# psy-ex/svt-av1-psy

Hardware: NVIDIA B200
Metric: 1080p preset-8 encoded frames/sec at 1/2/4/8 B200 vs reference AVX2 on host (higher is better)
Workload: dtype u8

## Files before the change

svt-av1-psy_b200/csrc/wiener.cu:

```cuda
#include <cuda_fp16.h>

#include <map>

#include "common.cuh"
#include "wiener_unit.cuh"
#include "../../include/svt_b200.h"
#include "wiener_stats_lag.cuh"

namespace b200 {


template <typename PIX>
__global__ void __launch_bounds__(256)
wiener_convolve_kernel(const PIX* __restrict__ src_base, PIX* __restrict__ dst_base, const SvtB200WienerUnit* __restrict__ units,
                       int n_units, int bd, int round0, int round1, int lbd_rows) {
    __shared__ __align__(16) uint16_t s_src[(64 + 8) * (64 + 8)];
    __shared__ __align__(16) uint16_t s_tmp[(64 + 8) * 64];
    for (int it = blockIdx.x; it < n_units; it += gridDim.x) {
        const SvtB200WienerUnit u = units[it];
        const int w = u.w, h = u.h;
        const PIX* src = src_base + u.src_off;
        PIX*       dst = dst_base + u.dst_off;
        const int sw = w + 8, sh = h + 7;
#pragma unroll 4
        for (int i = threadIdx.x; i < sw * sh; i += blockDim.x) {
            const int r = i / sw, c = i - r * sw;
            s_src[r * 72 + c] = (uint16_t)src[(ptrdiff_t)(r - 3) * u.src_stride + (c - 3)];
        }
        __syncthreads();
        wiener_unit_compute<PIX>(s_src, s_tmp, dst, u.dst_stride, w, h, u.hfilter, u.vfilter, bd, round0, round1, lbd_rows);
    }
}

constexpr int kSumParts = 16;
template <typename PIX>
__global__ void __launch_bounds__(256)
stats_sum_kernel(const PIX* __restrict__ dgd_base, const SvtB200StatsItem* __restrict__ items, unsigned long long* __restrict__ tot_out) {
    const int it = blockIdx.x / kSumParts, part = blockIdx.x % kSumParts;
    const SvtB200StatsItem s = items[it];
    const int w = s.h_end - s.h_start, h = s.v_end - s.v_start;
    const int warp = threadIdx.x >> 5, lane = threadIdx.x & 31;
    unsigned int acc = 0;
    unsigned long long wide = 0;
    for (int r = part * 8 + warp; r < h; r += kSumParts * 8) {
        const PIX* row = dgd_base + s.dgd_off + (ptrdiff_t)(s.v_start + r) * s.dgd_stride + s.h_start;
        for (int c = lane; c < w; c += 32) acc += row[c];
        if (acc > 0xf0000000u) { wide += acc; acc = 0; }
    }
    wide += acc;
#pragma unroll
    for (int o = 16; o > 0; o >>= 1) wide += __shfl_xor_sync(0xffffffffu, wide, o);
    if (lane == 0 && wide) atomicAdd(&tot_out[it], wide);
}

__device__ __forceinline__ int stats_average(const unsigned long long* tot, int it, const SvtB200StatsItem& s) {
    return (int)(tot[it] / (unsigned long long)((s.h_end - s.h_start) * (s.v_end - s.v_start)));
}

constexpr int kStatsMaxParts = 32;


constexpr int kMmaWarps = 4;
constexpr int kMmaTW = 64, kMmaTH = 32;
constexpr int kMmaPitch = 100;
constexpr int kMmaPRows = kMmaTH + 8;
constexpr int kMmaXBase = kMmaPRows * kMmaPitch + 28;
constexpr int kMmaWords = kMmaXBase + kMmaTH * kMmaPitch;
constexpr int kMmaAccMax = 16 * 128;
constexpr int kMmaFoldPixels = 33025 - kMmaTW * kMmaTH;
static_assert(kMmaPitch % 32 == 4 && (kMmaPRows * kMmaPitch) % 32 == 0, "bank layout");
static_assert(kMmaTW + 6 <= kMmaPitch && kMmaAccMax <= 2450, "layout");

__device__ __forceinline__ void mma_16816_f16f32(float (&c)[4], uint32_t a0, uint32_t a1, uint32_t a2, uint32_t a3, uint32_t b0,
                                                 uint32_t b1) {
    asm volatile("mma.sync.aligned.m16n8k16.row.col.f32.f16.f16.f32 {%0,%1,%2,%3}, {%4,%5,%6,%7}, {%8,%9}, {%0,%1,%2,%3};\n"
                 : "+f"(c[0]), "+f"(c[1]), "+f"(c[2]), "+f"(c[3])
                 : "r"(a0), "r"(a1), "r"(a2), "r"(a3), "r"(b0), "r"(b1));
}

__device__ __forceinline__ uint32_t pack_pair_f16(int lo, int hi) {
    const uint32_t bits = 0x64006400u + (uint32_t)(lo + 256) + ((uint32_t)(hi + 256) << 16);
    const __half2  h    = __hsub2(*reinterpret_cast<const __half2*>(&bits), __float2half2_rn(1280.f));
    return *reinterpret_cast<const uint32_t*>(&h);
}

__host__ __device__ __forceinline__ int mma_tile_index(int win, int m, int n) { return m * win - m * (m - 1) + n - 2 * m; }
__device__ __forceinline__ int stats_mma_parts(const SvtB200StatsItem& s, int ctas_per_item) {
    const int tiles = ((s.h_end - s.h_start + kMmaTW - 1) / kMmaTW) * ((s.v_end - s.v_start + kMmaTH - 1) / kMmaTH);
    return tiles < ctas_per_item ? tiles : ctas_per_item;
}

template <int WIN>
__device__ __forceinline__ void stats_mma_body(const uint8_t* __restrict__ dgd, const uint8_t* __restrict__ src, const SvtB200StatsItem& s,
                                               const int avg, const int part, const int parts, long long* __restrict__ P,
                                               uint32_t* __restrict__ tile, int* __restrict__ s32) {
    constexpr int NT = WIN, MT = (WIN + 1) / 2, HALF = WIN / 2, OFF = 3 - HALF;
    constexpr int NTILES = MT * WIN - MT * (MT - 1);
    const int warp = threadIdx.x >> 5, lane = threadIdx.x & 31, g = lane >> 2, t = lane & 3;
    int boff[NT];
#pragma unroll
    for (int n = 0; n < NT; n++) boff[n] = (OFF + g) * kMmaPitch + OFF + n + t;
    if (g == 7) boff[0] = kMmaXBase + t;
    float acc[NTILES][4];
#pragma unroll
    for (int i = 0; i < NTILES; i++) acc[i][0] = acc[i][1] = acc[i][2] = acc[i][3] = 0.f;
    for (int i = threadIdx.x; i < NTILES * 128; i += kMmaWarps * 32) s32[i] = 0;
    __syncthreads();
    auto flush_regs = [&]() {
#pragma unroll
        for (int i = 0; i < NTILES; i++)
#pragma unroll
            for (int r = 0; r < 4; r++) {
                atomicAdd(&s32[(i * 4 + r) * 32 + lane], __float2int_rn(acc[i][r]));
                acc[i][r] = 0.f;
            }
    };
    const int W = s.h_end - s.h_start, H = s.v_end - s.v_start;
    const int ntx = (W + kMmaTW - 1) / kMmaTW, nty = (H + kMmaTH - 1) / kMmaTH;
    const int vlo = s.v_start - HALF, vhi = s.v_end + HALF, hlo = s.h_start - HALF, hhi = s.h_end + HALF;
    int  ksteps = 0, pending = 0;
    bool spilled = false;
    auto prefetch_tile = [&](int tl) {
        const int ty = tl / ntx, tx = tl - ty * ntx;
        const int r0 = s.v_start + ty * kMmaTH, c0 = s.h_start + tx * kMmaTW;
        for (int w = threadIdx.x; w < 2 * (kMmaPRows + 1) + kMmaTH; w += kMmaWarps * 32) {
            const uint8_t* p;
            if (w < 2 * (kMmaPRows + 1)) {
                const int row = min(max(r0 - 3 + (w >> 1), vlo), vhi - 1);
                const int col = (w & 1) ? min(c0 + kMmaTW + 2, hhi - 1) : max(c0 - 3, hlo);
                p = dgd + (ptrdiff_t)row * s.dgd_stride + col;
            } else {
                const int row = min(r0 + (w - 2 * (kMmaPRows + 1)), s.v_end - 1);
                p = src + (ptrdiff_t)row * s.src_stride + min(c0 + 32, s.h_end - 1);
            }
            asm volatile("prefetch.global.L1 [%0];" ::"l"(p));
        }
    };
    for (int tl = part; tl < ntx * nty; tl += parts) {
        const int ty = tl / ntx, tx = tl - ty * ntx;
        const int r0 = s.v_start + ty * kMmaTH, c0 = s.h_start + tx * kMmaTW;
        const int nrows = min(kMmaTH, s.v_end - r0), ncols = min(kMmaTW, s.h_end - c0);
        if (pending > kMmaFoldPixels) {
            flush_regs();
            ksteps = 0;
            __syncthreads();
            for (int i = threadIdx.x; i < NTILES * 128; i += kMmaWarps * 32) {
                P[i] = (spilled ? P[i] : 0) + s32[i];
                s32[i] = 0;
            }
            spilled = true;
            pending = 0;
        }
        __syncthreads();
        for (int w = threadIdx.x; w < (kMmaTW + 6) * 4; w += kMmaWarps * 32) {
            const int  seg = w / (kMmaTW + 6), c = w - seg * (kMmaTW + 6);
            const int  col = c0 - 3 + c;
            const bool cv = col >= hlo && col < hhi;
            const int  rbeg = seg * (kMmaPRows / 4);
            auto ld = [&](int rr) {
                const int row = r0 - 3 + rr;
                return (cv && row >= vlo && row < vhi) ? (int)dgd[(ptrdiff_t)row * s.dgd_stride + col] - avg : 0;
            };
            int lo = ld(rbeg);
#pragma unroll
            for (int k = 0; k < kMmaPRows / 4; k++) {
                const int hi = ld(rbeg + k + 1);
                tile[(rbeg + k) * kMmaPitch + c] = pack_pair_f16(lo, hi);
                lo = hi;
            }
        }
        for (int w = threadIdx.x; w < (kMmaTH / 2) * kMmaTW; w += kMmaWarps * 32) {
            const int  r = (w / kMmaTW) * 2, c = w % kMmaTW;
            const bool cv = c < ncols;
            const uint8_t* p = src + (ptrdiff_t)(r0 + r) * s.src_stride + c0 + c;
            const int lo = (cv && r < nrows) ? (int)p[0] - avg : 0;
            const int hi = (cv && r + 1 < nrows) ? (int)p[s.src_stride] - avg : 0;
            tile[kMmaXBase + r * kMmaPitch + c] = pack_pair_f16(lo, hi);
        }
        __syncthreads();
        if (tl + parts < ntx * nty) prefetch_tile(tl + parts);
        const int cgs = (ncols + 7) >> 3, nsteps = cgs * ((nrows + 1) >> 1);
        for (int st = warp; st < nsteps; st += kMmaWarps) {
            const int rp = st / cgs, px = (st - rp * cgs) * 8, py = rp * 2;
            const uint32_t* base = tile + py * kMmaPitch + px;
            const uint32_t rowmask = (py + 1 < nrows) ? 0xffffffffu : 0x0000ffffu;
            const uint32_t m0 = (px + t < ncols) ? rowmask : 0u, m1 = (px + t + 4 < ncols) ? rowmask : 0u;
            uint32_t f0[NT], f1[NT];
#pragma unroll
            for (int n = 0; n < NT; n++) {
                f0[n] = base[boff[n]];
                f1[n] = base[boff[n] + 4];
            }
#pragma unroll
            for (int m = 0; m < MT; m++) {
                constexpr int last = NT - 1;
                const int     lo = 2 * m, hi = 2 * m + 1 <= last ? 2 * m + 1 : last;
#pragma unroll
                for (int n = 2 * m; n < NT; n++)
                    mma_16816_f16f32(acc[m * WIN - m * (m - 1) + n - 2 * m], f0[lo], f0[hi], f1[lo], f1[hi], f0[n] & m0, f1[n] & m1);
            }
            if (++ksteps == 16) {
                flush_regs();
                ksteps = 0;
            }
        }
        pending += nrows * ncols;
    }
    flush_regs();
    __syncthreads();
    for (int i = threadIdx.x; i < NTILES * 128; i += kMmaWarps * 32) P[i] = (spilled ? P[i] : 0) + s32[i];
}

__global__ void __launch_bounds__(kMmaWarps * 32)
stats_mma_kernel(const uint8_t* __restrict__ dgd_base, const uint8_t* __restrict__ src_base, const SvtB200StatsItem* __restrict__ items,
                 const unsigned long long* __restrict__ tot_in, int ctas_per_item, long long* __restrict__ partial) {
    __shared__ uint32_t tile[kMmaWords];
    __shared__ int      s32[kMmaAccMax];
    const int it = blockIdx.x / ctas_per_item, part = blockIdx.x % ctas_per_item;
    const SvtB200StatsItem s = items[it];
    const int avg = stats_average(tot_in, it, s);
    if (part >= stats_mma_parts(s, ctas_per_item)) return;
    long long* P = partial + ((size_t)it * ctas_per_item + part) * 2450;
    const uint8_t* dgd = dgd_base + s.dgd_off;
    const uint8_t* src = src_base + s.src_off;
    if (s.wiener_win == 7) stats_mma_body<7>(dgd, src, s, avg, part, ctas_per_item, P, tile, s32);
    else if (s.wiener_win == 5) stats_mma_body<5>(dgd, src, s, avg, part, ctas_per_item, P, tile, s32);
    else stats_mma_body<3>(dgd, src, s, avg, part, ctas_per_item, P, tile, s32);
}

__global__ void __launch_bounds__(256)
stats_finalize_kernel(const long long* __restrict__ partial, int parts, const SvtB200StatsItem* __restrict__ items, int divider,
                      int mma_layout, long long* __restrict__ M_out, long long* __restrict__ H_out) {
    const int it = blockIdx.y, e = blockIdx.x * blockDim.x + threadIdx.x;
    const int win = items[it].wiener_win, win2 = win * win;
    if (e >= win2 * win2 + win2) return;
    const int used = mma_layout ? stats_mma_parts(items[it], parts) : parts;
    int       src;
    if (e < win2 * win2) {
        const int k = e / win2, l = e - k * win2;
        int ka = k / win, kq = k - ka * win, la = l / win, lq = l - la * win;
        if (mma_layout) {
            if (ka > la) {
                int x = ka; ka = la; la = x;
                x = kq; kq = lq; lq = x;
            }
            src = (mma_tile_index(win, ka >> 1, la) * 4 + (ka & 1) * 2 + (lq & 1)) * 32 + kq * 4 + (lq >> 1);
        } else {
            src = (ka <= la) ? k * win2 + l : l * win2 + k;
        }
    } else {
        const int k = e - win2 * win2, ka = k / win, kq = k - ka * win;
        src = mma_layout ? (mma_tile_index(win, 0, ka) * 4 + (kq & 1)) * 32 + 28 + (kq >> 1) : 2401 + k;
    }
    long long v = 0;
    for (int p = 0; p < used; p++) v += partial[((size_t)it * parts + p) * 2450 + src];
    if (e < win2 * win2) H_out[(size_t)it * 2401 + e] = v / divider;
    else M_out[(size_t)it * 49 + (e - win2 * win2)] = v / divider;
}

struct StatsScratch {
    long long*          acc = nullptr;
    unsigned long long* tot = nullptr;
    size_t              cap = 0;
};
static std::map<cudaStream_t, StatsScratch> g_stats;
static std::mutex g_stats_mu;
static ResetHook g_stats_reset([] { std::lock_guard<std::mutex> lk(g_stats_mu); g_stats.clear(); });

template <typename PIX, int WIN>
static void launch_lag_bulk(const PIX* d_dgd, const PIX* d_src, const SvtB200StatsItem* d_items, int n, int cpi, unsigned long long* acc,
                            cudaStream_t st) {
    constexpr size_t smem = lag_bulk_smem<PIX, WIN>();
    static int attr = -1;
    if (attr != epoch()) {
        if (smem > 48 * 1024)
            B200_CUDA_CHECK(cudaFuncSetAttribute(stats_lag_bulk_kernel<PIX, WIN>, cudaFuncAttributeMaxDynamicSharedMemorySize, (int)smem));
        attr = epoch();
    }
    stats_lag_bulk_kernel<PIX, WIN><<<dim3(cpi, n), 256, smem, st>>>(d_dgd, d_src, d_items, acc);
    B200_LAUNCH_CHECK();
}

template <typename PIX>
static void launch_stats_mma(const PIX* d_dgd, const PIX* d_src, const SvtB200StatsItem* d_items, int n, int bd, long long* d_M,
                             long long* d_H, long long* d_acc, unsigned long long* d_tot, cudaStream_t st);

template <typename PIX>
static void launch_stats(const PIX* d_dgd, const PIX* d_src, const SvtB200StatsItem* d_items, int n, int bd, long long* d_M,
                         long long* d_H, long long* d_acc, unsigned long long* d_tot, cudaStream_t st) {
    if constexpr (sizeof(PIX) == 1) return launch_stats_mma<PIX>(d_dgd, d_src, d_items, n, bd, d_M, d_H, d_acc, d_tot, st);
    const int divider = bd == 12 ? 16 : (bd == 10 ? 4 : 1);
    int cpi = (ctx().sm_count * 8) / (n > 0 ? n : 1);
    if (cpi < 1) cpi = 1;
    if (cpi > 64) cpi = 64;
    unsigned long long* acc = reinterpret_cast<unsigned long long*>(d_acc);
    B200_CUDA_CHECK(cudaMemsetAsync(d_tot, 0, (size_t)n * sizeof(unsigned long long), st));
    B200_CUDA_CHECK(cudaMemsetAsync(acc, 0, (size_t)n * kLagItemWords * sizeof(unsigned long long), st));
    stats_sum_kernel<PIX><<<n * kSumParts, 256, 0, st>>>(d_dgd, d_items, d_tot);
    B200_LAUNCH_CHECK();
    launch_lag_bulk<PIX, 7>(d_dgd, d_src, d_items, n, cpi, acc, st);
    launch_lag_bulk<PIX, 5>(d_dgd, d_src, d_items, n, cpi, acc, st);
    launch_lag_bulk<PIX, 3>(d_dgd, d_src, d_items, n, cpi, acc, st);
    stats_lag_edges_kernel<PIX><<<dim3(kLagEdge, n), 256, 0, st>>>(d_dgd, d_items, acc);
    B200_LAUNCH_CHECK();
    stats_lag_finalize_kernel<PIX><<<dim3((49 * 50 / 2 + 49 + 127) / 128, n), 128, 0, st>>>(d_dgd, d_items, acc, d_tot, divider, d_M, d_H);
    B200_LAUNCH_CHECK();
}

template <typename PIX>
static void launch_stats_mma(const PIX* d_dgd, const PIX* d_src, const SvtB200StatsItem* d_items, int n, int bd, long long* d_M,
                             long long* d_H, long long* d_acc, unsigned long long* d_tot, cudaStream_t st) {
    const int divider = bd == 12 ? 16 : (bd == 10 ? 4 : 1);
    int cpi = (ctx().sm_count * (sizeof(PIX) == 1 ? 6 : 4)) / (n > 0 ? n : 1);
    if (cpi < 1) cpi = 1;
    if (cpi > (sizeof(PIX) == 1 ? kStatsMaxParts : 16)) cpi = sizeof(PIX) == 1 ? kStatsMaxParts : 16;
    B200_CUDA_CHECK(cudaMemsetAsync(d_tot, 0, (size_t)n * sizeof(unsigned long long), st));
    stats_sum_kernel<PIX><<<n * kSumParts, 256, 0, st>>>(d_dgd, d_items, d_tot);
    B200_LAUNCH_CHECK();
    static_assert(sizeof(PIX) == 1, "the tensor-core statistics are the 8-bit path (high bit depth: wiener_stats_lag.cuh)");
    stats_mma_kernel<<<n * cpi, kMmaWarps * 32, 0, st>>>(d_dgd, d_src, d_items, d_tot, cpi, d_acc);
    B200_LAUNCH_CHECK();
    stats_finalize_kernel<<<dim3((2450 + 255) / 256, n), 256, 0, st>>>(d_acc, cpi, d_items, divider, sizeof(PIX) == 1, d_M, d_H);
    B200_LAUNCH_CHECK();
}

template <typename PIX>
static void stats_t1(int wiener_win, const PIX* dgd, const PIX* src, int h_start, int h_end, int v_start, int v_end, int dgd_stride,
                     int src_stride, int64_t* M, int64_t* H, int bd) {
    require_ready();
    const int half = wiener_win >> 1, win2 = wiener_win * wiener_win;
    const int w = h_end - h_start, h = v_end - v_start;
    const int dw = w + 2 * half, dh = h + 2 * half;
    LaneGuard l;
    size_t o_d = l->alloc((size_t)dw * dh * sizeof(PIX)), o_s = l->alloc((size_t)w * h * sizeof(PIX)), o_it = l->alloc(sizeof(SvtB200StatsItem));
    size_t in_end = l->used;
    size_t o_M = l->alloc(49 * 8), o_H = l->alloc(2401 * 8), o_acc = l->alloc((size_t)kStatsMaxParts * 2450 * 8), o_avg = l->alloc(16);
    for (int r = 0; r < dh; r++)
        memcpy(l->h<PIX>(o_d) + (size_t)r * dw, dgd + (ptrdiff_t)(v_start - half + r) * dgd_stride + h_start - half, dw * sizeof(PIX));
    for (int r = 0; r < h; r++) memcpy(l->h<PIX>(o_s) + (size_t)r * w, src + (ptrdiff_t)(v_start + r) * src_stride + h_start, w * sizeof(PIX));
    SvtB200StatsItem* it = l->h<SvtB200StatsItem>(o_it);
    memset(it, 0, sizeof(*it));
    it->dgd_off = (uint64_t)half * dw + half;
    it->src_off = 0;
    it->dgd_stride = dw;
    it->src_stride = w;
    it->h_start = 0;
    it->h_end = w;
    it->v_start = 0;
    it->v_end = h;
    it->wiener_win = wiener_win;
    l->h2d(0, in_end);
    launch_stats<PIX>(l->d<PIX>(o_d), l->d<PIX>(o_s), l->d<SvtB200StatsItem>(o_it), 1, bd, l->d<long long>(o_M), l->d<long long>(o_H),
                      l->d<long long>(o_acc), l->d<unsigned long long>(o_avg), l->stream);
    l->d2h(o_M, (o_H + 2401 * 8) - o_M);
    l->sync();
    memcpy(M, l->h<int64_t>(o_M), (size_t)win2 * 8);
    memcpy(H, l->h<int64_t>(o_H), (size_t)win2 * win2 * 8);
}

template <typename PIX>
static void wiener_t1(const PIX* src, ptrdiff_t src_stride, PIX* dst, ptrdiff_t dst_stride, const int16_t* fx, const int16_t* fy, int w,
                      int h, int round0, int round1, int bd, int lbd_rows) {
    require_ready();
    LaneGuard l;
    const int sw = w + 8, sh = h + 7;
    size_t o_s = l->alloc((size_t)sw * sh * sizeof(PIX)), o_u = l->alloc(sizeof(SvtB200WienerUnit));
    size_t in_end = l->used;
    size_t o_d = l->alloc((size_t)w * h * sizeof(PIX));
    for (int r = 0; r < sh; r++) memcpy(l->h<PIX>(o_s) + (size_t)r * sw, src + (ptrdiff_t)(r - 3) * src_stride - 3, sw * sizeof(PIX));
    SvtB200WienerUnit* u = l->h<SvtB200WienerUnit>(o_u);
    memset(u, 0, sizeof(*u));
    u->src_off = (uint64_t)3 * sw + 3;
    u->dst_off = 0;
    u->src_stride = sw;
    u->dst_stride = w;
    u->w = (uint16_t)w;
    u->h = (uint16_t)h;
    memcpy(u->hfilter, fx, 16);
    memcpy(u->vfilter, fy, 16);
    l->h2d(0, in_end);
    wiener_convolve_kernel<PIX><<<1, 256, 0, l->stream>>>(l->d<PIX>(o_s), l->d<PIX>(o_d), l->d<SvtB200WienerUnit>(o_u), 1, bd, round0, round1, lbd_rows);
    B200_LAUNCH_CHECK();
    l->d2h(o_d, (size_t)w * h * sizeof(PIX));
    l->sync();
    for (int r = 0; r < h; r++) memcpy(dst + (ptrdiff_t)r * dst_stride, l->h<PIX>(o_d) + (size_t)r * w, w * sizeof(PIX));
}

}

using namespace b200;

extern "C" void svt_b200_av1_wiener_convolve_add_src(const uint8_t* src, ptrdiff_t src_stride, uint8_t* dst, ptrdiff_t dst_stride,
                                                     const int16_t* filter_x, const int16_t* filter_y, int32_t w, int32_t h,
                                                     const SvtB200ConvolveParams* conv_params) {
    wiener_t1<uint8_t>(src, src_stride, dst, dst_stride, filter_x, filter_y, w, h, conv_params->round_0, conv_params->round_1, 8, 1);
}
extern "C" void svt_b200_av1_highbd_wiener_convolve_add_src(const uint16_t* src, ptrdiff_t src_stride, uint16_t* dst,
                                                            ptrdiff_t dst_stride, const int16_t* filter_x, const int16_t* filter_y,
                                                            int32_t w, int32_t h, const SvtB200ConvolveParams* conv_params, int32_t bd) {
    wiener_t1<uint16_t>(src, src_stride, dst, dst_stride, filter_x, filter_y, w, h, conv_params->round_0, conv_params->round_1, bd, 0);
}
extern "C" void svt_b200_av1_compute_stats(int32_t wiener_win, const uint8_t* dgd, const uint8_t* src, int32_t h_start, int32_t h_end,
                                           int32_t v_start, int32_t v_end, int32_t dgd_stride, int32_t src_stride, int64_t* M, int64_t* H) {
    stats_t1<uint8_t>(wiener_win, dgd, src, h_start, h_end, v_start, v_end, dgd_stride, src_stride, M, H, 8);
}
extern "C" void svt_b200_av1_compute_stats_highbd(int32_t wiener_win, const uint16_t* dgd, const uint16_t* src, int32_t h_start,
                                                  int32_t h_end, int32_t v_start, int32_t v_end, int32_t dgd_stride, int32_t src_stride,
                                                  int64_t* M, int64_t* H, int32_t bit_depth) {
    stats_t1<uint16_t>(wiener_win, dgd, src, h_start, h_end, v_start, v_end, dgd_stride, src_stride, M, H, bit_depth);
}

extern "C" int svt_b200_wiener_units_dev(const void* d_src, void* d_dst, const SvtB200WienerUnit* d_units, int n_units, int bit_depth,
                                         void* stream) {
    require_ready();
    if (n_units <= 0) return n_units == 0 ? SVT_B200_OK : SVT_B200_ERR_BAD_ARG;
    const int round0 = bit_depth == 12 ? 5 : 3, round1 = 14 - round0;
    cudaStream_t st = (cudaStream_t)stream;
    if (bit_depth > 8)
        wiener_convolve_kernel<uint16_t><<<grid_for(n_units, 4), 256, 0, st>>>((const uint16_t*)d_src, (uint16_t*)d_dst, d_units, n_units, bit_depth, round0, round1, 0);
    else
        wiener_convolve_kernel<uint8_t><<<grid_for(n_units, 4), 256, 0, st>>>((const uint8_t*)d_src, (uint8_t*)d_dst, d_units, n_units, 8, round0, round1, 1);
    B200_LAUNCH_CHECK();
    return SVT_B200_OK;
}

extern "C" int svt_b200_compute_stats_batch_dev(const void* d_dgd, const void* d_src, const SvtB200StatsItem* d_items, int n_items,
                                                int bit_depth, int64_t* d_M, int64_t* d_H, void* stream) {
    require_ready();
    if (n_items <= 0) return n_items == 0 ? SVT_B200_OK : SVT_B200_ERR_BAD_ARG;
    std::lock_guard<std::mutex> lk(g_stats_mu);
    StatsScratch& sc = g_stats[(cudaStream_t)stream];
    if ((size_t)n_items > sc.cap) {
        sc.cap = (size_t)n_items * 2;
        sc.acc = (long long*)scratch_alloc(sc.cap * kStatsMaxParts * 2450 * 8);
        sc.tot = (unsigned long long*)scratch_alloc(sc.cap * 8);
    }
    if (bit_depth > 8)
        launch_stats<uint16_t>((const uint16_t*)d_dgd, (const uint16_t*)d_src, d_items, n_items, bit_depth, (long long*)d_M, (long long*)d_H,
                               sc.acc, sc.tot, (cudaStream_t)stream);
    else
        launch_stats<uint8_t>((const uint8_t*)d_dgd, (const uint8_t*)d_src, d_items, n_items, 8, (long long*)d_M, (long long*)d_H, sc.acc,
                              sc.tot, (cudaStream_t)stream);
    return SVT_B200_OK;
}
```

svt-av1-psy_b200/pipeline.py:

```python
import ctypes as ct

import numpy as np

from . import dsp
from .dsp import lib


def _t(torch, arr, dtype=None):
    t = torch.from_numpy(np.ascontiguousarray(arr))
    return t.cuda(non_blocking=False)


class _Arena:

    def __init__(self, torch, specs, device):
        self.torch = torch
        off, self.slots = 0, {}
        for name, dtype, shape in specs:
            n = int(np.prod(shape)) * torch.empty(0, dtype=dtype).element_size()
            self.slots[name] = (off, n, dtype, tuple(shape))
            off = (off + n + 255) & ~255
        self.nbytes = off
        self.dev = torch.zeros(off, dtype=torch.uint8, device=device)
        self.host = torch.zeros(off, dtype=torch.uint8).pin_memory()
# ... 195 lines not shown
    def call_quant(self, s):
        rc = lib.svt_b200_quant_batch_dev(self.coeff.data_ptr(), self.qcoeff.data_ptr(), self.dqcoeff.data_ptr(), self.scan.data_ptr(), self.iscan.data_ptr(),
                                          self.qm.data_ptr(), self.quant_items.data_ptr(), len(self.wl.quant_items), self.eobs.data_ptr(), s)
        assert rc == 0

    def call_inv_txfm(self, s):
        rc = lib.svt_b200_inv_txfm_batch_dev(self.dqcoeff.data_ptr(), self.pred.data_ptr(), self.recon.data_ptr(), self.inv_items.data_ptr(),
                                             self.tx_counts, self.psz, s)
        assert rc == 0

    def cdef_frame(self, recon_flat):
        wl = self.wl
        f = dsp.CdefFrame()
        (f.recon_y, sy), (f.recon_cb, sc), (f.recon_cr, _) = self.plane_views(recon_flat, True)
        (f.src_y, ssy), (f.src_cb, ssc), (f.src_cr, _) = self.plane_views(self.cur_flat, False)
        f.recon_stride_y, f.recon_stride_c, f.src_stride_y, f.src_stride_c = sy, sc, ssy, ssc
        f.width, f.height, f.bit_depth, f.damping, f.subsampling_factor = wl.width, wl.height, self.bd, wl.cdef_damping, wl.cdef_subsampling
        return f

    def call_cdef_search(self, s):
        f = self.cdef_frame(self.recon)
        rc = lib.svt_b200_cdef_search_frame_dev(ct.byref(f), self.skip.data_ptr(), self.str_y.data_ptr(), self.str_uv.data_ptr(),
                                                len(self.wl.cdef_str_y), self.cdef_mse.data_ptr(), self.cdef_dir.data_ptr(),
                                                self.cdef_var.data_ptr(), s)
        assert rc == 0

    def call_cdef_apply(self, s):
        f = self.cdef_frame(self.recon)
        self.cdef_out.copy_(self.recon, non_blocking=True)
        (oy, sy), (ocb, sc), (ocr, _) = self.plane_views(self.cdef_out, True)
        rc = lib.svt_b200_cdef_apply_frame_dev(ct.byref(f), self.skip.data_ptr(), self.fb_idx.data_ptr(), self.app_y.data_ptr(),
                                               self.app_uv.data_ptr(), self.cdef_dir.data_ptr(), self.cdef_var.data_ptr(), oy, ocb, ocr, sy, sc, s)
        assert rc == 0

    def call_rest_extend(self, s):
        wl = self.wl
        if self._extents is None:
            off, _ = wl.padded_offsets()
            self._extents = (dsp.PlaneExtent * 3)()
            for p in range(3):
                th, st = wl.padded_shape(p)
                w, h = wl.plane_dims[p]
                self._extents[p] = dsp.PlaneExtent(self.cdef_out.data_ptr() + off[p] * self.psz, st, w, h, wl.PAD, wl.PAD, self.psz)
        assert lib.svt_b200_extend_planes_dev(self._extents, 3, s) == 0

    def call_wiener_stats(self, s):
        rc = lib.svt_b200_compute_stats_batch_dev(self.cdef_out.data_ptr(), self.cur_flat.data_ptr(), self.stats_items.data_ptr(),
                                                  len(self.wl.stats_items), self.bd, self.M.data_ptr(), self.Hm.data_ptr(), s)
        assert rc == 0

    def lr_planes(self):
        if self._lr_planes is None:
            wl = self.wl
            self._lr_planes = (dsp.LrPlane * 3)()
            rec, cdf, fin = self.plane_views(self.recon, True), self.plane_views(self.cdef_out, True), self.plane_views(self.final, True)
            src = self.plane_views(self.cur_flat, False)
            for p in range(3):
                w, h = wl.plane_dims[p]
                ss = 1 if p else 0
                self._lr_planes[p] = dsp.LrPlane(rec[p][0], cdf[p][0], fin[p][0], src[p][0], self.lr_above[p].data_ptr(), self.lr_below[p].data_ptr(),
                                                 rec[p][1], cdf[p][1], fin[p][1], src[p][1], wl.lr_boundary_stride(p), w, h, ss, ss, wl.lr_unit_size[p],
                                                 1)
            self._lr_unit_ptrs = (ct.c_void_p * 3)(*[u.data_ptr() for u in self.lr_units])
        return self._lr_planes

    def call_lr_boundaries(self, s):
        pl = self.lr_planes()
        assert lib.svt_b200_lr_save_boundary_lines_dev(pl, 3, 0, self.bd, s) == 0
        assert lib.svt_b200_lr_save_boundary_lines_dev(pl, 3, 1, self.bd, s) == 0

    def call_wiener_filter(self, s):
        pl = self.lr_planes()
        assert lib.svt_b200_lr_filter_frame_dev(pl, 3, self._lr_unit_ptrs, 0, self.bd, s) == 0

    STAGES = ("me", "tx", "cdef", "rest")
    CALLS = (("me_pyramid", "me", "downsample_2d_kernel+pad_plane_kernel"),
             ("me_search", "me", "me_b64_hme_kernel + fullpel_search_kernel + me_b64_finish_kernel"),
             ("txfm_trio", "tx", "trio_txfm_kernel<4..64> (residual + forward transform + quantise + inverse transform fused)"),
             ("pack_levels", "tx", "eob_chunk_sum_kernel+eob_offsets_kernel+pack_levels_kernel"),
             ("cdef_search", "cdef", "cdef_dir_kernel+cdef_search_kernel"),
             ("cdef_apply", "cdef", "cdef_apply_kernel"),
             ("lr_boundaries", "rest", "lr_save_boundary_kernel x2"),
             ("rest_extend", "rest", "pad_plane_kernel"),
             ("wiener_stats", "rest", "stats_sum_kernel+stats_mma_kernel+stats_finalize_kernel"),
             ("wiener_filter", "rest", "lr_filter_kernel (striped restoration of the whole picture)"))

    def _stage(self, stage, s):
        for name, st, _ in self.CALLS:
            if st == stage:
                getattr(self, "call_" + name)(s)

    def stage_me(self, s):
        self._stage("me", s)

    def stage_tx(self, s):
        self._stage("tx", s)

    def stage_cdef(self, s):
        self._stage("cdef", s)

    def stage_rest(self, s):
        self._stage("rest", s)

    def step(self, events=None):
        T = self.torch
        cur = T.cuda.current_stream()
        if events is not None:
            s = cur.cuda_stream
            for i, (name, _, _) in enumerate(self.CALLS):
                events[i].record()
                getattr(self, "call_" + name)(s)
            events[len(self.CALLS)].record()
            return
        if self._side is None:
            self._side, self._forked, self._joined = T.cuda.Stream(), T.cuda.Event(), T.cuda.Event()
        self._forked.record(cur)
        self._side.wait_event(self._forked)
        with T.cuda.stream(self._side):
            self._stage("me", self._side.cuda_stream)
            self._joined.record(self._side)
        for st in ("tx", "cdef", "rest"):
            self._stage(st, cur.cuda_stream)
        cur.wait_event(self._joined)
```

Baseline: 2725.

## Move 8-bit Wiener statistics to tcgen05 int8 MMA with TMEM accumulation

Replaces the mma.sync fp16 Wiener statistics path for 8-bit with tcgen05 int8 MMAs accumulating in tensor memory, using double-buffered shared-memory operands and mbarrier commits. Raw pixel products, row sums and pixel counts are accumulated and mean-centred in the finalize kernel, which removes the separate stats_sum pre-pass and its dependency on the average. Larger 128-wide tiles and overlap of operand build with MMA aim to cut the per-tile cost. This adds considerable complexity in descriptor setup, TMEM allocation and synchronisation, and stats are only a small part of the whole encode.

```diff
diff --git a/svt-av1-psy_b200/csrc/wiener.cu b/svt-av1-psy_b200/csrc/wiener.cu
--- a/svt-av1-psy_b200/csrc/wiener.cu
+++ b/svt-av1-psy_b200/csrc/wiener.cu
@@ -1,5 +1,3 @@
-#include <cuda_fp16.h>
-
 #include <map>
 
 #include "common.cuh"
@@ -53,209 +51,304 @@
     if (lane == 0 && wide) atomicAdd(&tot_out[it], wide);
 }
 
-__device__ __forceinline__ int stats_average(const unsigned long long* tot, int it, const SvtB200StatsItem& s) {
-    return (int)(tot[it] / (unsigned long long)((s.h_end - s.h_start) * (s.v_end - s.v_start)));
-}
-
 constexpr int kStatsMaxParts = 32;
 
-
-constexpr int kMmaWarps = 4;
-constexpr int kMmaTW = 64, kMmaTH = 32;
-constexpr int kMmaPitch = 100;
-constexpr int kMmaPRows = kMmaTH + 8;
-constexpr int kMmaXBase = kMmaPRows * kMmaPitch + 28;
-constexpr int kMmaWords = kMmaXBase + kMmaTH * kMmaPitch;
-constexpr int kMmaAccMax = 16 * 128;
-constexpr int kMmaFoldPixels = 33025 - kMmaTW * kMmaTH;
-static_assert(kMmaPitch % 32 == 4 && (kMmaPRows * kMmaPitch) % 32 == 0, "bank layout");
-static_assert(kMmaTW + 6 <= kMmaPitch && kMmaAccMax <= 2450, "layout");
-
-__device__ __forceinline__ void mma_16816_f16f32(float (&c)[4], uint32_t a0, uint32_t a1, uint32_t a2, uint32_t a3, uint32_t b0,
-                                                 uint32_t b1) {
-    asm volatile("mma.sync.aligned.m16n8k16.row.col.f32.f16.f16.f32 {%0,%1,%2,%3}, {%4,%5,%6,%7}, {%8,%9}, {%0,%1,%2,%3};\n"
-                 : "+f"(c[0]), "+f"(c[1]), "+f"(c[2]), "+f"(c[3])
-                 : "r"(a0), "r"(a1), "r"(a2), "r"(a3), "r"(b0), "r"(b1));
-}
-
-__device__ __forceinline__ uint32_t pack_pair_f16(int lo, int hi) {
-    const uint32_t bits = 0x64006400u + (uint32_t)(lo + 256) + ((uint32_t)(hi + 256) << 16);
-    const __half2  h    = __hsub2(*reinterpret_cast<const __half2*>(&bits), __float2half2_rn(1280.f));
-    return *reinterpret_cast<const uint32_t*>(&h);
-}
-
-__host__ __device__ __forceinline__ int mma_tile_index(int win, int m, int n) { return m * win - m * (m - 1) + n - 2 * m; }
+constexpr int kTcThreads = 128;
+constexpr int kTcTW = 128;
+__host__ __device__ constexpr int stats_block_rows(int win) { return (127 - 9 * (win - 1)) / 8 + 1; }
+__host__ __device__ constexpr int stats_tile_rows(int win) { return stats_block_rows(win) * (36 / stats_block_rows(win)); }
+constexpr int kTcGrpBytes = 8 * 128 + 16;
+constexpr int kTcGroups = 40;
+constexpr int kTcBufBytes = kTcGroups * kTcGrpBytes;
+constexpr int kTcRowSums = kTcGroups * 8;
+constexpr int kTcDumpPitch = 129;
+constexpr int kTcSmem = 2 * kTcBufBytes + 2 * kTcRowSums * 4 + 32;
+constexpr int kTcFoldPixels = 33025;
+constexpr int kTcTmemCols = 256;
+constexpr bool stats_tc_fits(int win) {
+    return stats_tile_rows(win) + win - 1 <= kTcGroups && stats_tile_rows(win) - stats_block_rows(win) + 16 <= kTcGroups;
+}
+static_assert(stats_tc_fits(7) && stats_tc_fits(5) && stats_tc_fits(3), "operand buffer");
+static_assert(128 * kTcDumpPitch * 4 <= 2 * kTcBufBytes, "D is read back through the operand buffers");
+static_assert(kTcBufBytes % 16 == 0 && kTcSmem < 227 * 1024 / 2, "two CTAs per SM (2 x 256 TMEM columns)");
+
+constexpr int kPartG = 0, kPartGx = 1225, kPartS = kPartGx + 49, kPartSx = kPartS + 49, kPartN = kPartSx + 1;
+constexpr int kStatsPartWords = kPartN + 1;
+constexpr size_t kStatsItemWords = (size_t)kStatsMaxParts * kStatsPartWords;
+static_assert(kStatsItemWords >= (size_t)kLagItemWords, "the lag path shares the scratch");
+
+__host__ __device__ __forceinline__ int stats_tri_index(int w2, int p, int q) { return p * w2 - p * (p - 1) / 2 + q - p; }
 __device__ __forceinline__ int stats_mma_parts(const SvtB200StatsItem& s, int ctas_per_item) {
-    const int tiles = ((s.h_end - s.h_start + kMmaTW - 1) / kMmaTW) * ((s.v_end - s.v_start + kMmaTH - 1) / kMmaTH);
+    const int th = stats_tile_rows(s.wiener_win);
+    const int tiles = ((s.h_end - s.h_start + kTcTW - 1) / kTcTW) * ((s.v_end - s.v_start + th - 1) / th);
     return tiles < ctas_per_item ? tiles : ctas_per_item;
 }
 
+__device__ __forceinline__ uint32_t tc_smem(const void* p) { return (uint32_t)__cvta_generic_to_shared(p); }
+__device__ __forceinline__ void tc_fence_before() { asm volatile("tcgen05.fence::before_thread_sync;" ::: "memory"); }
+__device__ __forceinline__ void tc_fence_after() { asm volatile("tcgen05.fence::after_thread_sync;" ::: "memory"); }
+__device__ __forceinline__ void tc_bar_wait(uint64_t* bar, uint32_t parity) {
+    uint32_t ok;
+    do {
+        asm volatile("{ .reg .pred p; mbarrier.try_wait.parity.shared::cta.b64 p, [%1], %2; selp.u32 %0, 1, 0, p; }"
+                     : "=r"(ok) : "r"(tc_smem(bar)), "r"(parity) : "memory");
+    } while (!ok);
+}
+__device__ __forceinline__ uint64_t tc_desc(uint32_t addr) {
+    return (uint64_t)((addr >> 4) & 0x3fffu) | ((uint64_t)(128 >> 4) << 16) | ((uint64_t)(kTcGrpBytes >> 4) << 32) | (1ull << 46);
+}
+template <int N>
+__host__ __device__ constexpr uint32_t tc_idesc() { return (2u << 4) | ((uint32_t)(N >> 3) << 17) | ((uint32_t)(128 >> 4) << 24); }
+__device__ __forceinline__ void tc_mma_i8(uint32_t tmem, uint64_t desc, uint32_t idesc, uint32_t accum) {
+    asm volatile("{ .reg .pred p; setp.ne.b32 p, %3, 0;\n\t"
+                 "tcgen05.mma.cta_group::1.kind::i8 [%0], %1, %1, %2, p; }"
+                 ::"r"(tmem), "l"(desc), "r"(idesc), "r"(accum) : "memory");
+}
+__device__ __forceinline__ void tc_ld16(uint32_t taddr, uint32_t (&v)[16]) {
+    asm volatile("tcgen05.ld.sync.aligned.32x32b.x16.b32 {%0,%1,%2,%3,%4,%5,%6,%7,%8,%9,%10,%11,%12,%13,%14,%15}, [%16];"
+                 : "=r"(v[0]), "=r"(v[1]), "=r"(v[2]), "=r"(v[3]), "=r"(v[4]), "=r"(v[5]), "=r"(v[6]), "=r"(v[7]), "=r"(v[8]),
+                   "=r"(v[9]), "=r"(v[10]), "=r"(v[11]), "=r"(v[12]), "=r"(v[13]), "=r"(v[14]), "=r"(v[15])
+                 : "r"(taddr) : "memory");
+    asm volatile("tcgen05.wait::ld.sync.aligned;" ::: "memory");
+}
+
 template <int WIN>
-__device__ __forceinline__ void stats_mma_body(const uint8_t* __restrict__ dgd, const uint8_t* __restrict__ src, const SvtB200StatsItem& s,
-                                               const int avg, const int part, const int parts, long long* __restrict__ P,
-                                               uint32_t* __restrict__ tile, int* __restrict__ s32) {
-    constexpr int NT = WIN, MT = (WIN + 1) / 2, HALF = WIN / 2, OFF = 3 - HALF;
-    constexpr int NTILES = MT * WIN - MT * (MT - 1);
-    const int warp = threadIdx.x >> 5, lane = threadIdx.x & 31, g = lane >> 2, t = lane & 3;
-    int boff[NT];
-#pragma unroll
-    for (int n = 0; n < NT; n++) boff[n] = (OFF + g) * kMmaPitch + OFF + n + t;
-    if (g == 7) boff[0] = kMmaXBase + t;
-    float acc[NTILES][4];
-#pragma unroll
-    for (int i = 0; i < NTILES; i++) acc[i][0] = acc[i][1] = acc[i][2] = acc[i][3] = 0.f;
-    for (int i = threadIdx.x; i < NTILES * 128; i += kMmaWarps * 32) s32[i] = 0;
+__device__ __forceinline__ void tc_build(uint8_t* __restrict__ op, int* __restrict__ rs, const uint8_t* __restrict__ dgd,
+                                         const uint8_t* __restrict__ src, int dgd_stride, int src_stride, int r0, int c0, int nrows,
+                                         int ncols) {
+    constexpr int HALF = WIN / 2;
+    constexpr uint32_t ONES = 0x01010101u;
+    const int ng = nrows + WIN - 1, nkc = ((ncols + 31) >> 5) * 2;
+    for (int c = threadIdx.x; c < ng * nkc; c += kTcThreads) {
+        const int kc = c / ng, g = c - kc * ng;
+        const int kv = min(max(ncols - 16 * kc, 0), 16);
+        uint32_t mask[4];
+#pragma unroll
+        for (int m = 0; m < 4; m++) {
+            const int vb = min(max(kv - 4 * m, 0), 4);
+            mask[m] = vb == 4 ? 0xffffffffu : (1u << (8 * vb)) - 1u;
+        }
+        uint8_t* dst = op + g * kTcGrpBytes + kc * 128;
+        int*     rsg = rs + g * 8;
+        const int r = r0 - HALF + g;
+        const uint8_t*  p   = dgd + (ptrdiff_t)r * dgd_stride + (c0 - HALF + 16 * kc);
+        const uint32_t  off = (uint32_t)(uintptr_t)p & 3u;
+        const uint32_t* wp  = reinterpret_cast<const uint32_t*>(p - off);
+        const int       nw  = kv ? (int)(off + kv + WIN + 2) >> 2 : 0;
+        uint32_t w[7], u[6];
+#pragma unroll
+        for (int i = 0; i < 7; i++) w[i] = i < nw ? __ldg(wp + i) : 0u;
+#pragma unroll
+        for (int i = 0; i < 6; i++) u[i] = __funnelshift_r(w[i], w[i + 1], off * 8);
+#pragma unroll
+        for (int dx = 0; dx < WIN; dx++) {
+            uint32_t o[4];
+#pragma unroll
+            for (int m = 0; m < 4; m++) o[m] = __funnelshift_r(u[(dx >> 2) + m], u[(dx >> 2) + m + 1], (dx & 3) * 8) & mask[m];
+            *reinterpret_cast<uint4*>(dst + dx * 16) = make_uint4(o[0], o[1], o[2], o[3]);
+            const uint32_t sum = __dp4a(o[0], ONES, __dp4a(o[1], ONES, __dp4a(o[2], ONES, __dp4a(o[3], ONES, 0u))));
+            if (sum) atomicAdd(&rsg[dx], (int)sum);
+        }
+        if (g >= HALF && g < HALF + nrows) {
+            const uint8_t*  q    = src + (ptrdiff_t)r * src_stride + c0 + 16 * kc;
+            const uint32_t  off2 = (uint32_t)(uintptr_t)q & 3u;
+            const uint32_t* wq   = reinterpret_cast<const uint32_t*>(q - off2);
+            const int       nw2  = kv ? (int)(off2 + kv + 3) >> 2 : 0;
+            uint32_t x[5], o[4];
+#pragma unroll
+            for (int i = 0; i < 5; i++) x[i] = i < nw2 ? __ldg(wq + i) : 0u;
+#pragma unroll
+            for (int m = 0; m < 4; m++) o[m] = __funnelshift_r(x[m], x[m + 1], off2 * 8) & mask[m];
+            *reinterpret_cast<uint4*>(dst + 7 * 16) = make_uint4(o[0], o[1], o[2], o[3]);
+            const uint32_t sum = __dp4a(o[0], ONES, __dp4a(o[1], ONES, __dp4a(o[2], ONES, __dp4a(o[3], ONES, 0u))));
+            if (sum) atomicAdd(&rsg[7], (int)sum);
+        }
+    }
+}
+
+template <int WIN>
+__device__ __forceinline__ void stats_tc_body(const uint8_t* __restrict__ dgd, const uint8_t* __restrict__ src, const SvtB200StatsItem& s,
+                                              const int part, const int parts, long long* __restrict__ P, uint8_t* smem) {
+    constexpr int HALF = WIN / 2, W2 = WIN * WIN, T = stats_block_rows(WIN), TH = stats_tile_rows(WIN);
+    constexpr uint32_t IDESC = tc_idesc<128>();
+    static_assert((TH - 1 + WIN - 1) * 8 + 7 < kTcRowSums, "row sums of a tile");
+    int*      rsum  = reinterpret_cast<int*>(smem + 2 * kTcBufBytes);
+    uint64_t* bar   = reinterpret_cast<uint64_t*>(rsum + 2 * kTcRowSums);
+    uint32_t* tslot = reinterpret_cast<uint32_t*>(bar + 2);
+    const int tid = threadIdx.x, warp = tid >> 5;
+    if (tid == 0) {
+        asm volatile("mbarrier.init.shared::cta.b64 [%0], 1;" ::"r"(tc_smem(&bar[0])) : "memory");
+        asm volatile("mbarrier.init.shared::cta.b64 [%0], 1;" ::"r"(tc_smem(&bar[1])) : "memory");
+        asm volatile("fence.mbarrier_init.release.cluster;" ::: "memory");
+    }
+    for (int i = tid; i < 2 * kTcRowSums; i += kTcThreads) rsum[i] = 0;
+    if (warp == 0) {
+        asm volatile("tcgen05.alloc.cta_group::1.sync.aligned.shared::cta.b32 [%0], %1;" ::"r"(tc_smem(tslot)), "r"(kTcTmemCols) : "memory");
+        asm volatile("tcgen05.relinquish_alloc_permit.cta_group::1.sync.aligned;" ::: "memory");
+    }
+    tc_fence_before();
     __syncthreads();
-    auto flush_regs = [&]() {
-#pragma unroll
-        for (int i = 0; i < NTILES; i++)
-#pragma unroll
-            for (int r = 0; r < 4; r++) {
-                atomicAdd(&s32[(i * 4 + r) * 32 + lane], __float2int_rn(acc[i][r]));
-                acc[i][r] = 0.f;
+    tc_fence_after();
+    const uint32_t tmem = *tslot;
+
+    const int W = s.h_end - s.h_start, H = s.v_end - s.v_start;
+    const int ntx = (W + kTcTW - 1) / kTcTW, nty = (H + TH - 1) / TH, ntiles = ntx * nty;
+    const int rlast = (H - (nty - 1) * TH) % T;
+    auto drain_one = [&](uint32_t col, int nt, bool add) {
+        int* d = reinterpret_cast<int*>(smem);
+#pragma unroll 1
+        for (int c = 0; c < 128; c += 16) {
+            uint32_t v[16];
+            tc_ld16(tmem + ((uint32_t)(warp * 32) << 16) + col + (uint32_t)c, v);
+#pragma unroll
+            for (int j = 0; j < 16; j++) d[tid * kTcDumpPitch + c + j] = (int)v[j];
+        }
+        __syncthreads();
+        for (int e = tid; e < W2 * W2 + W2; e += kTcThreads) {
+            int p, b;
+            long long* dst;
+            if (e < W2 * W2) {
+                p = e / W2;
+                const int q = e - p * W2;
+                if (q < p) continue;
+                b   = 8 * (q % WIN) + q / WIN;
+                dst = P + kPartG + stats_tri_index(W2, p, q);
+            } else {
+                p   = e - W2 * W2;
+                b   = 8 * HALF + 7;
+                dst = P + kPartGx + p;
             }
+            const int  a = 8 * (p % WIN) + p / WIN;
+            long long  g = 0;
+            const int* dd = d + a * kTcDumpPitch + b;
+            for (int t = 0; t < nt; t++) g += dd[t * (8 * kTcDumpPitch + 8)];
+            *dst = (add ? *dst : 0) + g;
+        }
+        __syncthreads();
     };
-    const int W = s.h_end - s.h_start, H = s.v_end - s.v_start;
-    const int ntx = (W + kMmaTW - 1) / kMmaTW, nty = (H + kMmaTH - 1) / kMmaTH;
-    const int vlo = s.v_start - HALF, vhi = s.v_end + HALF, hlo = s.h_start - HALF, hhi = s.h_end + HALF;
-    int  ksteps = 0, pending = 0;
-    bool spilled = false;
-    auto prefetch_tile = [&](int tl) {
+    bool full_used = false, part_used = false;
+    auto drain = [&](bool add) {
+        if (full_used) {
+            drain_one(0, T, add);
+            add = true;
+        }
+        if (part_used) drain_one(128, rlast, add);
+    };
+
+    const int  dy = tid >> 3, dx = tid & 7, pidx = dx * WIN + dy;
+    const bool wlane = dy < WIN && dx < WIN, slane = wlane || tid == 8 * HALF + 7;
+    long long  ssum = 0, npix = 0;
+    int        pending = 0;
+    bool       spilled = false;
+    uint32_t   inflight = 0, phase = 0;
+    auto wait_buf = [&](int b) {
+        if (inflight >> b & 1u) {
+            tc_bar_wait(&bar[b], phase >> b & 1u);
+            phase ^= 1u << b;
+            inflight &= ~(1u << b);
+        }
+    };
+    for (int tl = part, j = 0; tl < ntiles; tl += parts, j++) {
+        const int b  = j & 1;
         const int ty = tl / ntx, tx = tl - ty * ntx;
-        const int r0 = s.v_start + ty * kMmaTH, c0 = s.h_start + tx * kMmaTW;
-        for (int w = threadIdx.x; w < 2 * (kMmaPRows + 1) + kMmaTH; w += kMmaWarps * 32) {
-            const uint8_t* p;
-            if (w < 2 * (kMmaPRows + 1)) {
-                const int row = min(max(r0 - 3 + (w >> 1), vlo), vhi - 1);
-                const int col = (w & 1) ? min(c0 + kMmaTW + 2, hhi - 1) : max(c0 - 3, hlo);
-                p = dgd + (ptrdiff_t)row * s.dgd_stride + col;
-            } else {
-                const int row = min(r0 + (w - 2 * (kMmaPRows + 1)), s.v_end - 1);
-                p = src + (ptrdiff_t)row * s.src_stride + min(c0 + 32, s.h_end - 1);
+        const int r0 = s.v_start + ty * TH, c0 = s.h_start + tx * kTcTW;
+        const int nrows = min(TH, s.v_end - r0), ncols = min(kTcTW, s.h_end - c0);
+        __syncthreads();
+        if (pending + nrows * ncols > kTcFoldPixels) {
+            wait_buf(b ^ 1);
+            tc_fence_after();
+            drain(spilled);
+            tc_fence_before();
+            spilled   = true;
+            full_used = part_used = false;
+            pending   = 0;
+        }
+        wait_buf(b);
+        uint8_t* op = smem + b * kTcBufBytes;
+        int*     rs = rsum + b * kTcRowSums;
+        tc_build<WIN>(op, rs, dgd, src, s.dgd_stride, s.src_stride, r0, c0, nrows, ncols);
+        asm volatile("fence.proxy.async.shared::cta;" ::: "memory");
+        __syncthreads();
+        if (tid == 0) {
+            tc_fence_after();
+            const uint64_t d0 = tc_desc(tc_smem(op));
+            const int      nk = (ncols + 31) >> 5;
+            for (int y = 0; y < nrows; y += T) {
+                const bool full = y + T <= nrows;
+                bool&      used = full ? full_used : part_used;
+                for (int k = 0; k < nk; k++) {
+                    tc_mma_i8(tmem + (full ? 0u : 128u), d0 + (uint64_t)((y * kTcGrpBytes + k * 256) >> 4), IDESC, used ? 1u : 0u);
+                    used = true;
+                }
             }
-            asm volatile("prefetch.global.L1 [%0];" ::"l"(p));
-        }
-    };
-    for (int tl = part; tl < ntx * nty; tl += parts) {
-        const int ty = tl / ntx, tx = tl - ty * ntx;
-        const int r0 = s.v_start + ty * kMmaTH, c0 = s.h_start + tx * kMmaTW;
-        const int nrows = min(kMmaTH, s.v_end - r0), ncols = min(kMmaTW, s.h_end - c0);
-        if (pending > kMmaFoldPixels) {
-            flush_regs();
-            ksteps = 0;
-            __syncthreads();
-            for (int i = threadIdx.x; i < NTILES * 128; i += kMmaWarps * 32) {
-                P[i] = (spilled ? P[i] : 0) + s32[i];
-                s32[i] = 0;
-            }
-            spilled = true;
-            pending = 0;
+            asm volatile("tcgen05.commit.cta_group::1.mbarrier::arrive::one.shared::cluster.b64 [%0];" ::"r"(tc_smem(&bar[b])) : "memory");
+        } else {
+            if (nrows >= T) full_used = true;
+            if (nrows % T) part_used = true;
+        }
+        inflight |= 1u << b;
+        if (slane) {
+            int t = 0;
+            for (int y = 0; y < nrows; y++) t += rs[(y + dy) * 8 + dx];
+            ssum += t;
         }
         __syncthreads();
-        for (int w = threadIdx.x; w < (kMmaTW + 6) * 4; w += kMmaWarps * 32) {
-            const int  seg = w / (kMmaTW + 6), c = w - seg * (kMmaTW + 6);
-            const int  col = c0 - 3 + c;
-            const bool cv = col >= hlo && col < hhi;
-            const int  rbeg = seg * (kMmaPRows / 4);
-            auto ld = [&](int rr) {
-                const int row = r0 - 3 + rr;
-                return (cv && row >= vlo && row < vhi) ? (int)dgd[(ptrdiff_t)row * s.dgd_stride + col] - avg : 0;
-            };
-            int lo = ld(rbeg);
-#pragma unroll
-            for (int k = 0; k < kMmaPRows / 4; k++) {
-                const int hi = ld(rbeg + k + 1);
-                tile[(rbeg + k) * kMmaPitch + c] = pack_pair_f16(lo, hi);
-                lo = hi;
-            }
-        }
-        for (int w = threadIdx.x; w < (kMmaTH / 2) * kMmaTW; w += kMmaWarps * 32) {
-            const int  r = (w / kMmaTW) * 2, c = w % kMmaTW;
-            const bool cv = c < ncols;
-            const uint8_t* p = src + (ptrdiff_t)(r0 + r) * s.src_stride + c0 + c;
-            const int lo = (cv && r < nrows) ? (int)p[0] - avg : 0;
-            const int hi = (cv && r + 1 < nrows) ? (int)p[s.src_stride] - avg : 0;
-            tile[kMmaXBase + r * kMmaPitch + c] = pack_pair_f16(lo, hi);
-        }
-        __syncthreads();
-        if (tl + parts < ntx * nty) prefetch_tile(tl + parts);
-        const int cgs = (ncols + 7) >> 3, nsteps = cgs * ((nrows + 1) >> 1);
-        for (int st = warp; st < nsteps; st += kMmaWarps) {
-            const int rp = st / cgs, px = (st - rp * cgs) * 8, py = rp * 2;
-            const uint32_t* base = tile + py * kMmaPitch + px;
-            const uint32_t rowmask = (py + 1 < nrows) ? 0xffffffffu : 0x0000ffffu;
-            const uint32_t m0 = (px + t < ncols) ? rowmask : 0u, m1 = (px + t + 4 < ncols) ? rowmask : 0u;
-            uint32_t f0[NT], f1[NT];
-#pragma unroll
-            for (int n = 0; n < NT; n++) {
-                f0[n] = base[boff[n]];
-                f1[n] = base[boff[n] + 4];
-            }
-#pragma unroll
-            for (int m = 0; m < MT; m++) {
-                constexpr int last = NT - 1;
-                const int     lo = 2 * m, hi = 2 * m + 1 <= last ? 2 * m + 1 : last;
-#pragma unroll
-                for (int n = 2 * m; n < NT; n++)
-                    mma_16816_f16f32(acc[m * WIN - m * (m - 1) + n - 2 * m], f0[lo], f0[hi], f1[lo], f1[hi], f0[n] & m0, f1[n] & m1);
-            }
-            if (++ksteps == 16) {
-                flush_regs();
-                ksteps = 0;
-            }
-        }
+        for (int i = tid; i < kTcRowSums; i += kTcThreads) rs[i] = 0;
         pending += nrows * ncols;
-    }
-    flush_regs();
+        npix += nrows * ncols;
+    }
+    wait_buf(0);
+    wait_buf(1);
+    tc_fence_after();
+    drain(spilled);
+    if (wlane) P[kPartS + pidx] = ssum;
+    if (tid == 8 * HALF + 7) P[kPartSx] = ssum;
+    if (tid == 0) P[kPartN] = npix;
+    tc_fence_before();
     __syncthreads();
-    for (int i = threadIdx.x; i < NTILES * 128; i += kMmaWarps * 32) P[i] = (spilled ? P[i] : 0) + s32[i];
-}
-
-__global__ void __launch_bounds__(kMmaWarps * 32)
+    if (warp == 0) {
+        tc_fence_after();
+        asm volatile("tcgen05.dealloc.cta_group::1.sync.aligned.b32 %0, %1;" ::"r"(tmem), "r"(kTcTmemCols) : "memory");
+    }
+}
+
+__global__ void __launch_bounds__(kTcThreads)
 stats_mma_kernel(const uint8_t* __restrict__ dgd_base, const uint8_t* __restrict__ src_base, const SvtB200StatsItem* __restrict__ items,
-                 const unsigned long long* __restrict__ tot_in, int ctas_per_item, long long* __restrict__ partial) {
-    __shared__ uint32_t tile[kMmaWords];
-    __shared__ int      s32[kMmaAccMax];
+                 int ctas_per_item, long long* __restrict__ partial) {
+    extern __shared__ __align__(1024) uint8_t smem[];
     const int it = blockIdx.x / ctas_per_item, part = blockIdx.x % ctas_per_item;
     const SvtB200StatsItem s = items[it];
-    const int avg = stats_average(tot_in, it, s);
     if (part >= stats_mma_parts(s, ctas_per_item)) return;
-    long long* P = partial + ((size_t)it * ctas_per_item + part) * 2450;
+    long long* P = partial + ((size_t)it * ctas_per_item + part) * kStatsPartWords;
     const uint8_t* dgd = dgd_base + s.dgd_off;
     const uint8_t* src = src_base + s.src_off;
-    if (s.wiener_win == 7) stats_mma_body<7>(dgd, src, s, avg, part, ctas_per_item, P, tile, s32);
-    else if (s.wiener_win == 5) stats_mma_body<5>(dgd, src, s, avg, part, ctas_per_item, P, tile, s32);
-    else stats_mma_body<3>(dgd, src, s, avg, part, ctas_per_item, P, tile, s32);
+    if (s.wiener_win == 7) stats_tc_body<7>(dgd, src, s, part, ctas_per_item, P, smem);
+    else if (s.wiener_win == 5) stats_tc_body<5>(dgd, src, s, part, ctas_per_item, P, smem);
+    else stats_tc_body<3>(dgd, src, s, part, ctas_per_item, P, smem);
 }
 
 __global__ void __launch_bounds__(256)
-stats_finalize_kernel(const long long* __restrict__ partial, int parts, const SvtB200StatsItem* __restrict__ items, int divider,
-                      int mma_layout, long long* __restrict__ M_out, long long* __restrict__ H_out) {
+stats_finalize_kernel(const long long* __restrict__ partial, int parts, const SvtB200StatsItem* __restrict__ items,
+                      long long* __restrict__ M_out, long long* __restrict__ H_out) {
     const int it = blockIdx.y, e = blockIdx.x * blockDim.x + threadIdx.x;
-    const int win = items[it].wiener_win, win2 = win * win;
-    if (e >= win2 * win2 + win2) return;
-    const int used = mma_layout ? stats_mma_parts(items[it], parts) : parts;
-    int       src;
-    if (e < win2 * win2) {
-        const int k = e / win2, l = e - k * win2;
-        int ka = k / win, kq = k - ka * win, la = l / win, lq = l - la * win;
-        if (mma_layout) {
-            if (ka > la) {
-                int x = ka; ka = la; la = x;
-                x = kq; kq = lq; lq = x;
-            }
-            src = (mma_tile_index(win, ka >> 1, la) * 4 + (ka & 1) * 2 + (lq & 1)) * 32 + kq * 4 + (lq >> 1);
-        } else {
-            src = (ka <= la) ? k * win2 + l : l * win2 + k;
-        }
+    const int win = items[it].wiener_win, w2 = win * win;
+    if (e >= w2 * w2 + w2) return;
+    const int        used = stats_mma_parts(items[it], parts);
+    const long long* P    = partial + (size_t)it * parts * kStatsPartWords;
+    auto total = [&](int w) {
+        long long v = 0;
+        for (int p = 0; p < used; p++) v += P[(size_t)p * kStatsPartWords + w];
+        return v;
+    };
+    const long long n = total(kPartN), v = total(kPartS + w2 / 2) / n, nvv = n * v * v;
+    if (e < w2 * w2) {
+        const int k = e / w2, l = e - k * w2;
+        const long long g = total(kPartG + stats_tri_index(w2, min(k, l), max(k, l)));
+        H_out[(size_t)it * 2401 + e] = g - v * (total(kPartS + k) + total(kPartS + l)) + nvv;
     } else {
-        const int k = e - win2 * win2, ka = k / win, kq = k - ka * win;
-        src = mma_layout ? (mma_tile_index(win, 0, ka) * 4 + (kq & 1)) * 32 + 28 + (kq >> 1) : 2401 + k;
-    }
-    long long v = 0;
-    for (int p = 0; p < used; p++) v += partial[((size_t)it * parts + p) * 2450 + src];
-    if (e < win2 * win2) H_out[(size_t)it * 2401 + e] = v / divider;
-    else M_out[(size_t)it * 49 + (e - win2 * win2)] = v / divider;
+        const int k = e - w2 * w2;
+        M_out[(size_t)it * 49 + k] = total(kPartGx + k) - v * (total(kPartS + k) + total(kPartSx)) + nvv;
+    }
 }
 
 struct StatsScratch {
@@ -281,14 +374,26 @@
     B200_LAUNCH_CHECK();
 }
 
-template <typename PIX>
-static void launch_stats_mma(const PIX* d_dgd, const PIX* d_src, const SvtB200StatsItem* d_items, int n, int bd, long long* d_M,
-                             long long* d_H, long long* d_acc, unsigned long long* d_tot, cudaStream_t st);
+static void launch_stats_mma(const uint8_t* d_dgd, const uint8_t* d_src, const SvtB200StatsItem* d_items, int n, long long* d_M,
+                             long long* d_H, long long* d_acc, cudaStream_t st) {
+    int cpi = (ctx().sm_count * 6) / (n > 0 ? n : 1);
+    if (cpi < 1) cpi = 1;
+    if (cpi > kStatsMaxParts) cpi = kStatsMaxParts;
+    static int attr = -1;
+    if (attr != epoch()) {
+        B200_CUDA_CHECK(cudaFuncSetAttribute(stats_mma_kernel, cudaFuncAttributeMaxDynamicSharedMemorySize, kTcSmem));
+        attr = epoch();
+    }
+    stats_mma_kernel<<<n * cpi, kTcThreads, kTcSmem, st>>>(d_dgd, d_src, d_items, cpi, d_acc);
+    B200_LAUNCH_CHECK();
+    stats_finalize_kernel<<<dim3((2450 + 255) / 256, n), 256, 0, st>>>(d_acc, cpi, d_items, d_M, d_H);
+    B200_LAUNCH_CHECK();
+}
 
 template <typename PIX>
 static void launch_stats(const PIX* d_dgd, const PIX* d_src, const SvtB200StatsItem* d_items, int n, int bd, long long* d_M,
                          long long* d_H, long long* d_acc, unsigned long long* d_tot, cudaStream_t st) {
-    if constexpr (sizeof(PIX) == 1) return launch_stats_mma<PIX>(d_dgd, d_src, d_items, n, bd, d_M, d_H, d_acc, d_tot, st);
+    if constexpr (sizeof(PIX) == 1) return launch_stats_mma(d_dgd, d_src, d_items, n, d_M, d_H, d_acc, st);
     const int divider = bd == 12 ? 16 : (bd == 10 ? 4 : 1);
     int cpi = (ctx().sm_count * 8) / (n > 0 ? n : 1);
     if (cpi < 1) cpi = 1;
@@ -304,23 +409,6 @@
     stats_lag_edges_kernel<PIX><<<dim3(kLagEdge, n), 256, 0, st>>>(d_dgd, d_items, acc);
     B200_LAUNCH_CHECK();
     stats_lag_finalize_kernel<PIX><<<dim3((49 * 50 / 2 + 49 + 127) / 128, n), 128, 0, st>>>(d_dgd, d_items, acc, d_tot, divider, d_M, d_H);
-    B200_LAUNCH_CHECK();
-}
-
-template <typename PIX>
-static void launch_stats_mma(const PIX* d_dgd, const PIX* d_src, const SvtB200StatsItem* d_items, int n, int bd, long long* d_M,
-                             long long* d_H, long long* d_acc, unsigned long long* d_tot, cudaStream_t st) {
-    const int divider = bd == 12 ? 16 : (bd == 10 ? 4 : 1);
-    int cpi = (ctx().sm_count * (sizeof(PIX) == 1 ? 6 : 4)) / (n > 0 ? n : 1);
-    if (cpi < 1) cpi = 1;
-    if (cpi > (sizeof(PIX) == 1 ? kStatsMaxParts : 16)) cpi = sizeof(PIX) == 1 ? kStatsMaxParts : 16;
-    B200_CUDA_CHECK(cudaMemsetAsync(d_tot, 0, (size_t)n * sizeof(unsigned long long), st));
-    stats_sum_kernel<PIX><<<n * kSumParts, 256, 0, st>>>(d_dgd, d_items, d_tot);
-    B200_LAUNCH_CHECK();
-    static_assert(sizeof(PIX) == 1, "the tensor-core statistics are the 8-bit path (high bit depth: wiener_stats_lag.cuh)");
-    stats_mma_kernel<<<n * cpi, kMmaWarps * 32, 0, st>>>(d_dgd, d_src, d_items, d_tot, cpi, d_acc);
-    B200_LAUNCH_CHECK();
-    stats_finalize_kernel<<<dim3((2450 + 255) / 256, n), 256, 0, st>>>(d_acc, cpi, d_items, divider, sizeof(PIX) == 1, d_M, d_H);
     B200_LAUNCH_CHECK();
 }
 
@@ -334,7 +422,7 @@
     LaneGuard l;
     size_t o_d = l->alloc((size_t)dw * dh * sizeof(PIX)), o_s = l->alloc((size_t)w * h * sizeof(PIX)), o_it = l->alloc(sizeof(SvtB200StatsItem));
     size_t in_end = l->used;
-    size_t o_M = l->alloc(49 * 8), o_H = l->alloc(2401 * 8), o_acc = l->alloc((size_t)kStatsMaxParts * 2450 * 8), o_avg = l->alloc(16);
+    size_t o_M = l->alloc(49 * 8), o_H = l->alloc(2401 * 8), o_acc = l->alloc(kStatsItemWords * 8), o_avg = l->alloc(16);
     for (int r = 0; r < dh; r++)
         memcpy(l->h<PIX>(o_d) + (size_t)r * dw, dgd + (ptrdiff_t)(v_start - half + r) * dgd_stride + h_start - half, dw * sizeof(PIX));
     for (int r = 0; r < h; r++) memcpy(l->h<PIX>(o_s) + (size_t)r * w, src + (ptrdiff_t)(v_start + r) * src_stride + h_start, w * sizeof(PIX));
@@ -432,7 +520,7 @@
     StatsScratch& sc = g_stats[(cudaStream_t)stream];
     if ((size_t)n_items > sc.cap) {
         sc.cap = (size_t)n_items * 2;
-        sc.acc = (long long*)scratch_alloc(sc.cap * kStatsMaxParts * 2450 * 8);
+        sc.acc = (long long*)scratch_alloc(sc.cap * kStatsItemWords * 8);
         sc.tot = (unsigned long long*)scratch_alloc(sc.cap * 8);
     }
     if (bit_depth > 8)
diff --git a/svt-av1-psy_b200/pipeline.py b/svt-av1-psy_b200/pipeline.py
--- a/svt-av1-psy_b200/pipeline.py
+++ b/svt-av1-psy_b200/pipeline.py
@@ -301,7 +301,7 @@
              ("cdef_apply", "cdef", "cdef_apply_kernel"),
              ("lr_boundaries", "rest", "lr_save_boundary_kernel x2"),
              ("rest_extend", "rest", "pad_plane_kernel"),
-             ("wiener_stats", "rest", "stats_sum_kernel+stats_mma_kernel+stats_finalize_kernel"),
+             ("wiener_stats", "rest", "stats_mma_kernel+stats_finalize_kernel (8-bit; 10-bit: stats_sum_kernel+stats_lag_*)"),
              ("wiener_filter", "rest", "lr_filter_kernel (striped restoration of the whole picture)"))
 
     def _stage(self, stage, s):
```

Result: faster. 3017, median of 6 (+10.7%).
